# craabreu/openmm-nonbonded-slicing

Measured on AMD Instinct MI355X. Metric: ns/day (force evaluation only, dt = 2 fs), higher is better.
Workload: dtype f32

## Files before the change

### openmm-nonbonded-slicing_amd/csrc/engine.hip

```cpp
#include "../../include/snb.h"
#include "snb_internal.h"
#include "switches.h"
#include "host_lists.h"
#include "ewald_fit.h"
#include "pme_sizes.h"
#include "pair_addressing.h"

#include <algorithm>
#include <cstdio>
#include <cstdlib>
#include <chrono>
#include <cmath>
#include <cstring>
#include <map>
#include <numeric>
#include <set>
#include <thread>
#include <tuple>
#include <type_traits>

namespace snb {

static thread_local std::string g_createError;

// ... 138 lines not shown

static void bsplineModuli(int n, int order, std::vector<double>& out) {
    std::vector<double> data(order, 0.0), bsp(std::max(n, order + 1), 0.0);
    data[order - 1] = 0; data[1] = 0; data[0] = 1;
    for (int k = 3; k < order; k++) {
        double div = 1.0 / (k - 1.0);
        data[k - 1] = 0;
        for (int l = 1; l < (k - 1); l++) data[k - l - 1] = div * (l * data[k - l - 2] + (k - l) * data[k - l - 1]);
        data[0] = div * data[0];
    }
    double div = 1.0 / (order - 1);
    data[order - 1] = 0;
    for (int l = 1; l < (order - 1); l++) data[order - l - 1] = div * (l * data[order - l - 2] + (order - l) * data[order - l - 1]);
    data[0] = div * data[0];
    for (int i = 1; i <= order; i++) bsp[i] = data[i - 1];
    out.assign(n, 0.0);
    for (int i = 0; i < n; i++) {
        double sc = 0, ss = 0;
        for (int j = 0; j < n && j <= order; j++) { double arg = (2.0 * SNB_PI * i * j) / n; sc += bsp[j] * std::cos(arg); ss += bsp[j] * std::sin(arg); }
        out[i] = sc * sc + ss * ss;
    }
    for (int i = 0; i < n; i++)
        if (out[i] < 1.0e-7) out[i] = (out[(i - 1 + n) % n] + out[(i + 1) % n]) / 2;
}

template <typename Real> struct PmePlan {
    PmePlanDims d;
    double alpha = 0;
    bool dispersion = false;
    DevBuf<Real> gridReal;
    DevBuf<typename Vec<Real>::T2> gridCplx, gridCplxB, twx, twy, twz;
    DevBuf<Real> modx, mody, modz;
    DevBuf<Real> planeEterm; bool planeEtermReady = false, planeEtermFilled = false; double planeEtermKey[10] = {0};
    int ownSlabs = 0, ownMargin = 1; DevBuf<unsigned char> ownPartial; DevBuf<int> ownBusy; DevBuf<int2> strays;
    void init(const int g[3], int nGrids, hipStream_t s) {
        if (!planDims(g, sizeof(Real), switches(), d)) throw HipError{"PME mesh size is not FFT-legal"};
        if (d.nx > 1024 || d.ny > 1024 || d.nz > 1024) throw HipError{"PME mesh dimensions above 1024 are not supported"};
        gridReal.resize((size_t)nGrids * d.nx * d.ny * d.nz);
        gridCplx.resize((size_t)nGrids * d.nx * d.ny * d.nzc);
        if (planePath(d, nGrids, sizeof(Real), switches()).buffers) { gridCplxB.resize((size_t)nGrids * d.nx * (d.ny + 8) * d.nzc);
             planeEterm.resize((size_t)d.nx * d.ny * d.nzc); planeEtermReady = false; }
        auto tw = [&](int n, DevBuf<typename Vec<Real>::T2>& buf) {
            std::vector<typename Vec<Real>::T2> h(n);
            for (int k = 0; k < n; k++) { double a = -2.0 * SNB_PI * k / n; h[k].x = (Real)std::cos(a); h[k].y = (Real)std::sin(a); }
            buf.upload(h, s);
        };
        tw(d.nx, twx); tw(d.ny, twy); tw(d.nz, twz);
        auto md = [&](int n, DevBuf<Real>& buf) {
            std::vector<double> m; bsplineModuli(n, SNB_PME_ORDER, m);
            std::vector<Real> h(m.begin(), m.end());
            buf.upload(h, s);
        };
        md(d.nx, modx); md(d.ny, mody); md(d.nz, modz);
        HIPCHECK(hipStreamSynchronize(s));
    }
};

template <typename Real> class Engine : public EngineBase {
    using T4 = typename Vec<Real>::T4;
    using T2 = typename Vec<Real>::T2;
public:
    int N, nsub, S;
    hipStream_t stream = nullptr; bool ownStream = false;
    static constexpr int RING = 32;
    hipEvent_t evRebuild[3] = {nullptr, nullptr, nullptr};
    hipEvent_t evStepDone[2] = {nullptr, nullptr}; long long stepCounter = 0;
    hipStream_t stream2 = nullptr; hipEvent_t evFork = nullptr, evJoin = nullptr, evPairA = nullptr;
// ... 206 lines not shown
        HIPCHECK(hipHostMalloc((void**)&hNbPub, 64, hipHostMallocMapped));
        std::memset(hNbPub, 0, 64);
        HIPCHECK(hipHostGetDevicePointer((void**)&dNbPub, hNbPub, 0));
        for (int s = 0; s < nsub; s++) if (s % cfg.shard_count == cfg.shard_rank) ownedSubsets.push_back(s);
        nGrids = cfg.shard_count == 1 ? nsub : (int)ownedSubsets.size();
        if (isPme()) {
            for (int d = 0; d < 3; d++) cfg.grid[d] = legalGridSize(cfg.grid[d]);
            pme.alpha = cfg.alpha; pme.dispersion = false;
            if (nGrids > 0) pme.init(cfg.grid, nGrids, stream); else { pme.d.nx = cfg.grid[0]; pme.d.ny = cfg.grid[1]; pme.d.nz = cfg.grid[2]; }
            if (cfg.method == SNB_LJPME) {
                for (int d = 0; d < 3; d++) cfg.dgrid[d] = legalGridSize(cfg.dgrid[d]);
                dpme.alpha = cfg.alpha_d; dpme.dispersion = true;
                if (nGrids > 0) dpme.init(cfg.dgrid, nGrids, stream); else { dpme.d.nx = cfg.dgrid[0]; dpme.d.ny = cfg.dgrid[1]; dpme.d.nz = cfg.dgrid[2]; }
            }
            std::vector<int> gs = cfg.shard_count == 1 ? std::vector<int>() : ownedSubsets;
            if (cfg.shard_count == 1) { gs.resize(nsub); std::iota(gs.begin(), gs.end(), 0); }
            gridSubset.upload(gs, stream);
            hostGridSubset = gs;
        }
    }
    ~Engine() override {
        (void)hipStreamSynchronize(stream);
        if (sw.verbose && stats.n_rebuilds > 0) fprintf(stderr, "[snb] rebuilds: %lld, of them %lld built beside the steps; %lld side builds discarded\n", (long long)stats.n_rebuilds, sideBuilds, sideDiscarded);
        if (dStepTrace.p) {
            long long t[16] = {0}; (void)hipMemcpy(t, dStepTrace.p, sizeof(t), hipMemcpyDeviceToHost);
            auto us = [&](int k) { return t[k] ? (t[k] - t[0]) / 100.0 : -1.0; };
            fprintf(stderr, "[snb] step trace (us after the gather pass started; -1: not run): pair A %.1f .. %.1f | pair B %.1f .. %.1f | own %.1f | merge %.1f | plane %.1f | mix+z %.1f .. %.1f | interpolation %.1f .. %.1f\n",
                    us(2), us(3), us(4), us(5), us(6), us(7), us(8), us(9), us(10), us(11), us(12));
        }
        if (dPmeTrace.p) {
            long long g[8] = {0}; (void)hipMemcpy(g, dPmeTrace.p, 64, hipMemcpyDeviceToHost);
            if (g[7] > 0 && g[3] > 0) fprintf(stderr, "[snb] merge kernel prologue (busy flags, roots of unity, barrier): %.2f us per busy work-group\n", g[3] / 100.0 / g[7]);
            if (g[7] > 0) fprintf(stderr, "[snb] spreading (busy work-groups; scanning spreader: scan / entries / z FFT + store; merge kernel: sums / strays + z FFT / store): %.2f us, %.2f us, %.2f us per work-group (%lld work-groups)\n", g[4] / 100.0 / g[7], g[5] / 100.0 / g[7], g[6] / 100.0 / g[7], g[7]);
        }
        if (dPmeTrace.p) { long long h[4] = {0, 0, 0, 0}; (void)hipMemcpy(h, dPmeTrace.p, 32, hipMemcpyDeviceToHost); if (h[2] > 0) fprintf(stderr, "[snb] interpolation bricks: mean load %.2f us, mean compute %.2f us per work-group (%lld work-groups)\n", h[0] / 100.0 / h[2], h[1] / 100.0 / h[2], h[2]); }
        destroyGraphs();
        if (streamBuild) { (void)hipStreamSynchronize(streamBuild); (void)hipStreamDestroy(streamBuild); if (evSnap) (void)hipEventDestroy(evSnap); if (evBuilt) (void)hipEventDestroy(evBuilt); if (evFlagsReset) (void)hipEventDestroy(evFlagsReset); }
        if (streamCopy) { (void)hipStreamSynchronize(streamCopy); (void)hipStreamDestroy(streamCopy); }
        for (int k = 0; k < 2; k++) { if (evFrameStep[k]) (void)hipEventDestroy(evFrameStep[k]); if (evFrameUp[k]) (void)hipEventDestroy(evFrameUp[k]); if (framePinned[k]) (void)hipHostFree(framePinned[k]); }
        if (evBatchStart) (void)hipEventDestroy(evBatchStart);
        for (auto& g : sortGraphs) if (g.exec) (void)hipGraphExecDestroy(g.exec);
        sortGraphs.clear();
        for (auto& r : ring) { for (int k = 0; k < 5; k++) (void)hipEventDestroy(r.e[k]); for (int k = 0; k < 16; k++) { (void)hipEventDestroy(r.ks.start[k]); (void)hipEventDestroy(r.ks.stop[k]); } }
        for (int k = 0; k < 3; k++) if (evRebuild[k]) (void)hipEventDestroy(evRebuild[k]);
        for (int k = 0; k < 2; k++) if (evStepDone[k]) (void)hipEventDestroy(evStepDone[k]);
        if (hDispFlags) (void)hipHostFree(hDispFlags);
        if (hNbPub) (void)hipHostFree(hNbPub);
        if (stream2) { (void)hipEventDestroy(evFork); (void)hipEventDestroy(evJoin); (void)hipEventDestroy(evPairA); (void)hipStreamDestroy(stream2); }
        if (ownStream) (void)hipStreamDestroy(stream);
    }
    static constexpr int EW_DEG = sizeof(Real) == 4 ? 11 : SNB_EW_DEG_F64;
    static_assert(kEwaldFitLJPME == SNB_LJPME && kEwDegF32 == 11 && kEwDegF64 == SNB_EW_DEG_F64 && kDispDegF64 == SNB_DISP_DEG_F64, "ewald_fit.h and the kernels disagree");
    static_assert(kPolyForce == SNB_POLY_FORCE && kPolyEnergy == SNB_POLY_ENERGY && kPolyDispersion == SNB_POLY_DISPERSION, "ewald_fit.h and the kernels disagree");
    double ewPoly[EW_DEG + 1] = {0}; double ewPolyE[14] = {0}; double dispPoly[21] = {0}; double ewR2Max = 1;
    int polyMask = 0;
    void buildEwaldPoly() {
        const double rmax = cfg.cutoff + std::max(cfg.neighbor_padding, 0.0) + 0.02;
        const EwaldFit fit = fitEwaldPolys<Real>(cfg.alpha, cfg.alpha_d, cfg.cutoff, rmax, cfg.method);
        ewR2Max = fit.r2max;
        for (int i = 0; i <= EW_DEG; i++) ewPoly[i] = fit.ewPoly[i];
        for (int i = 0; i < 14; i++) ewPolyE[i] = fit.ewPolyE[i];
        for (int i = 0; i < 21; i++) dispPoly[i] = fit.dispPoly[i];
        const int have = sizeof(Real) == 4 ? (SNB_POLY_FORCE | SNB_POLY_ENERGY) : (SNB_POLY_FORCE | (cfg.method == SNB_LJPME ? SNB_POLY_DISPERSION : 0));
        polyMask = sw.ewaldErfc ? 0 : (sw.ewaldPolyAlways ? have : (fit.use & have));
        if (sw.verbose) fprintf(stderr, "[snb] Ewald polynomials: force max r|dBt| %.3g (limit %.3g), energy |dEt| %.3g (%.3g), dispersion max r|dGd| %.3g (%.3g): mask %d in use\n", fit.pairF, fit.limF, fit.sysE, fit.limE, fit.pairD, fit.limD, polyMask);
    }
// ... 511 lines not shown
            if (predicted && (h[7] > Npad || h[7] < N || (h[7] & 31))) {
                if (h[7] < N || (h[7] & 31)) throw HipError{"neighbour build: inconsistent padded atom count"};
                npadPredict = 0; padMispredictions++;
                if (sw.verbose) fprintf(stderr, "[snb] rebuild: padded count %d exceeded the predicted %d, repeating with the exact count (%lld so far)\n", h[7], Npad, (long long)padMispredictions);
                return gpuRebuild();
            }
            if (nbTrace && h[3] == 0) {
                std::vector<long long> tr((size_t)4 * numBlocks);
                HIPCHECK(hipMemcpy(tr.data(), dNbTrace.p, sizeof(long long) * tr.size(), hipMemcpyDeviceToHost));
                long long t0min = tr[0], t1max = tr[1]; std::vector<long long> dur(numBlocks);
                tr.resize((size_t)4 * numBlocks);
                for (int b = 0; b < numBlocks; b++) { t0min = std::min(t0min, tr[2 * b]); t1max = std::max(t1max, tr[2 * b + 1]); dur[b] = tr[2 * b + 1] - tr[2 * b]; }
                std::vector<long long> sorted = dur; std::sort(sorted.begin(), sorted.end());
                fprintf(stderr, "[snb] nb trace: span %.1f us; per-block duration median %.1f us, p90 %.1f, p99 %.1f, max %.1f us; last start at %.1f us\n", (t1max - t0min) / 100.0, sorted[numBlocks / 2] / 100.0,
                        sorted[numBlocks * 9 / 10] / 100.0, sorted[numBlocks * 99 / 100] / 100.0, sorted.back() / 100.0, (t1max - t0min) / 100.0);
                { std::vector<long long> a(numBlocks), b(numBlocks), c(numBlocks);
                  for (int k = 0; k < numBlocks; k++) { a[k] = tr[2 * numBlocks + 2 * k] - tr[2 * k]; b[k] = tr[2 * numBlocks + 2 * k + 1] - tr[2 * numBlocks + 2 * k]; c[k] = tr[2 * k + 1] - tr[2 * numBlocks + 2 * k + 1]; }
                  std::sort(a.begin(), a.end()); std::sort(b.begin(), b.end()); std::sort(c.begin(), c.end());
                  fprintf(stderr, "[snb] nb trace: median prologue %.1f us, gather %.1f us, final flush %.1f us\n", a[numBlocks / 2] / 100.0, b[numBlocks / 2] / 100.0, c[numBlocks / 2] / 100.0); }
                long long lastStart = 0; for (int b = 0; b < numBlocks; b++) lastStart = std::max(lastStart, tr[2 * b] - t0min);
                fprintf(stderr, "[snb] nb trace: last block start %.1f us after the first\n", lastStart / 100.0);
            }
            if (h[3] == 0) { acceptBuild(h, sortMs); gpuBuilt = true; needRebuild = false; paramsDirty = false; stepsSinceRebuild = 0; (void)t0; return true; }
            if (sw.verbose) fprintf(stderr, "[snb] gpu neighbour build attempt %d: tiles %d work %d masks %d overflow %d partial %d maxPartTiles %d maxPartWork %d (cap %zu, region %zu / %zu)\n", attempt, h[0], h[1], h[2], h[3], h[4], h[5], h[6], tileCap, tileCap / 64, (tileCap / 4 + 2 * numBlocks + 64) / 64);
            if ((size_t)h[5] > tileCap / 64 || (size_t)h[6] > (tileCap / 4 + 2 * numBlocks + 64) / 64) { tileCap = std::max((size_t)h[5] * 64 * 5 / 4, tileCap * 3 / 2) + 4096; continue; }
            return false;
        }
        return false;
    }

    void fillPme(PmeParams<Real>& p, PmePlan<Real>& plan, bool wantEnergy, const int* need, bool cellsReady = false, bool trace = false) {
        p.d = plan.d; p.nsub = nGrids; p.natoms = Npad; p.posq = posq.p; p.sigeps = sigeps.p; p.atomSubset = atomSubset.p; p.atomGrid = atomGrid.p;
        p.cells = pmeCells.p;
        if (sw.pmeTrace) { if (!dPmeTrace.p) { dPmeTrace.resize(8); HIPCHECK(hipMemset(dPmeTrace.p, 0, 64)); } p.trace = dPmeTrace.p; }
        p.stepTrace = (trace && plan.dispersion == (cfg.method == SNB_LJPME)) ? dStepTrace.p : nullptr;
        p.cellsReady = (!plan.dispersion && cellsReady) ? 1 : 0;
        p.fixDev = dFixScale.p ? dFixScale.p + (plan.dispersion ? 2 : 0) : nullptr;
        p.gridReal = plan.gridReal.p; p.gridCplx = plan.gridCplx.p; p.planeB = plan.gridCplxB.p; p.planeEterm = plan.planeEtermReady ? plan.planeEterm.p : nullptr; p.twx = plan.twx.p; p.twy = plan.twy.p; p.twz = plan.twz.p;
        p.modx = plan.modx.p; p.mody = plan.mody.p; p.modz = plan.modz.p;
        const double det = box[0] * box[4] * box[8];
        double r[9]; recipBoxRows(box, r);
        for (int i = 0; i < 9; i++) { p.recip[i] = (Real)r[i]; p.recipLo[i] = (Real)(r[i] - (double)p.recip[i]); }
        p.alpha = (Real)plan.alpha; p.volume = (Real)det; p.dispersion = plan.dispersion ? 1 : 0;
        p.lambdas = dLambdas.p; p.sliceNeed = need; p.gridSubset = gridSubset.p; p.emptyGrids = emptyGrids; p.nsubTotal = nsub; p.mix = cfg.shard_count == 1 ? 1 : 0;
        p.mix16 = sw.mix16 ? 1 : 0;
        p.sliceE = sliceE.p; p.fpx = fpx.p; p.fpy = fpy.p; p.fpz = fpz.p; p.wantEnergy = wantEnergy ? 1 : 0;
        p.sortNcx = p.sortNcy = 0; p.groupX = p.groupY = 1; p.colRange = nullptr;
        p.zSlabs = 1;
        if (plan.d.nz % 2 == 0 && plan.d.nz >= 32 && !(sizeof(Real) == 4)) p.zSlabs = 2;
        if (sw.zSlabs >= 1 && plan.d.nz % sw.zSlabs == 0) p.zSlabs = sw.zSlabs;
        const BrickGeometry b = bricksFor(plan);
        if (b.ok) {
            p.sortNcx = b.ncx; p.sortNcy = b.ncy; p.groupX = b.gx; p.groupY = b.gy; p.colRange = colRange.p;
            p.ownSlabs = plan.ownSlabs; p.ownMargin = plan.ownMargin; p.ownPartial = plan.ownPartial.p; p.ownBusy = plan.ownBusy.p;
            p.strays = plan.strays.p; p.strayCount = dStrayCount.p ? dStrayCount.p + (plan.dispersion ? 1 : 0) : nullptr;
            if (!p.ownPartial || !p.ownBusy || !p.strays || !p.strayCount) p.ownSlabs = 0;
        }
    }
    BrickGeometry bricksFor(const PmePlan<Real>& plan) const { return brickGeometry(plan.d, pme.d, colCells, sw.brickGroup); }
    void planPlaneTable(PmePlan<Real>& plan) {
        if (!plan.planeEterm.p || !plan.gridCplxB.p || nGrids <= 0) { plan.planeEtermReady = false; return; }
        double key[10]; for (int i = 0; i < 9; i++) key[i] = box[i]; key[9] = plan.alpha;
        if (plan.planeEtermReady && plan.planeEtermFilled && std::memcmp(key, plan.planeEtermKey, sizeof(key)) == 0) return;
        std::memcpy(plan.planeEtermKey, key, sizeof(key));
        plan.planeEtermReady = false;
        PmeParams<Real> pp; std::memset(&pp, 0, sizeof(pp));
        fillPme(pp, plan, false, dSliceNeedAll.p);
        plan.planeEtermFilled = launchPlaneEterm<Real>(pp, plan.planeEterm.p, stream);
        plan.planeEtermReady = true;
    }
    void describeMesh(const char* name, const PmePlan<Real>& plan) const {
        const BrickGeometry b = bricksFor(plan);
        const bool bricks = nGrids > 0 && b.ok;
        fprintf(stderr, "[snb] %s mesh %d x %d x %d: sort columns %d x %d of %d x %d cells, %s", name, plan.d.nx, plan.d.ny, plan.d.nz,
                colCells[0] > 0 ? pme.d.nx / colCells[0] : 0, colCells[0] > 0 ? pme.d.ny / colCells[1] : 0, colCells[0], colCells[1],
                !bricks ? "atomic spreader" : "");
        if (bricks) fprintf(stderr, "bricks of %d x %d columns, %s (slabs %d, margin %d)", b.gx, b.gy, plan.ownSlabs > 0 ? "own-atoms spreader planned" : "scanning brick spreader", plan.ownSlabs, plan.ownMargin);
        const PmePlanDims& d = plan.d;
        fprintf(stderr, "; fft splits x %d*%d y %d*%d z %d*%d, plane splits x %d*%d y %d*%d (%s)\n", d.rx1, d.rx2, d.ry1, d.ry2, d.rz1, d.rz2, d.px1, d.px2, d.py1, d.py2,
                (d.px1 <= 0 || d.py1 <= 0) ? "none" : planeIsStatic(d) ? "static" : "run-time");
    }
    void planOwnSpread(PmePlan<Real>& plan) {
        plan.ownSlabs = 0;
        const BrickGeometry b = bricksFor(plan);
        if (nGrids <= 0 || !b.ok) return;
        double r[9]; recipBoxRows(box, r);
        const int M = ownSpreadMargin(plan.d, r, cfg.neighbor_padding, sw);
        const OwnSpread o = ownSpread(plan.d, b, nGrids, sizeof(Real), M, sw);
        if (!o.slabs) return;
        plan.ownPartial.resize(o.partialBytes);
        plan.ownBusy.resize(o.regions); plan.strays.resize(std::max(Npad, 1));
        plan.ownSlabs = o.slabs; plan.ownMargin = M;
    }

    void checkBox(const double* x, bool recip, const std::string& prefix, bool kmax) {
        const double minAllowed = 1.999999 * cfg.cutoff;
        if (x && !(x[0] >= minAllowed && x[4] >= minAllowed && x[8] >= minAllowed)) { err = prefix + "The periodic box size has decreased to less than twice the nonbonded cutoff."; throw (int)SNB_ERR_BOX_TOO_SMALL; }
        if (cfg.method != SNB_Ewald || !recip) return;
        if (kmax && (cfg.kmax[0] < 1 || cfg.kmax[1] < 1 || cfg.kmax[2] < 1)) { err = "Ewald: kmax must be given explicitly (snb_config.kmax)"; throw (int)SNB_ERR_INVALID_ARGUMENT; }
        if (x && (x[3] != 0 || x[6] != 0 || x[7] != 0)) { err = prefix + "SlicedNonbondedForce: Ewald is not supported with non-rectangular boxes.  Use PME instead."; throw (int)SNB_ERR_UNSUPPORTED; }
    }
    bool beginExecute(bool forces, int includeRecip) {
        if (!haveParticles) throw HipError{"snb_execute: particles were not set"};
        if (!havePositions) throw HipError{"snb_execute: positions were not set"};
        if (isPeriodic()) {
            if (!haveBox) throw HipError{"snb_execute: box was not set"};
            checkBox(box, includeRecip != 0, "", true);
        }
        if (dLambdas.p == nullptr) setLambdas(lambdas.data());
        const bool autoMode = cfg.rebuild_interval < 0;
        if (autoMode && cfg.neighbor_padding > 0) {
            hipEvent_t& ev = evStepDone[stepCounter & 1];
            if (ev) HIPCHECK(hipEventSynchronize(ev));
        }
        if (flagsResetPending && hipEventQuery(evFlagsReset) == hipSuccess) flagsResetPending = false;
        const bool due = autoMode ? ((hDispFlags[0] != 0 && !flagsResetPending) || stepsSinceRebuild >= -cfg.rebuild_interval) : (cfg.rebuild_interval <= 1 || stepsSinceRebuild >= cfg.rebuild_interval);
        bool rebuilding = needRebuild || paramsDirty || due || cfg.neighbor_padding <= 0;
        if (!forces && rebuilding) keepLastForces();
        if (sidePending) {
            if (needRebuild || paramsDirty || staticDirty || valuesDirty || excValuesDirty || cfg.neighbor_padding <= 0) cancelSideBuild();
            else if (rebuilding && finishSideBuild()) rebuilding = false;
        }
        if ((valuesDirty || excValuesDirty) && !staticDirty && !rebuilding) refreshValues();
        if (rebuilding) { if (valuesDirty || excValuesDirty) { staticDirty = true; valuesDirty = excValuesDirty = false; } if (ctx.on) stageCtxPositions(ctxStage.p); rebuild(); }
// ... 978 lines not shown
```

### openmm-nonbonded-slicing_amd/csrc/pme.hip

```cpp
#include "snb_internal.h"
#include "switches.h"
#include "pme_sizes.h"
#include "pme_plan.h"
#include <cstdio>
#include <cstdlib>
#include <type_traits>
#include <algorithm>
#include <cstdlib>

namespace snb {

thread_local KernelStamps* g_stamps = nullptr;
template <typename Real> static inline int stampSlot(const PmeParams<Real>& p, int k) { return k + (p.dispersion ? 8 : 0); }

template <typename... KArgs, typename... Args>
static void launchLds(int slot, void (*kernel)(KArgs...), dim3 grid, dim3 block, size_t lds, hipStream_t s, const Args&... args) {
    hipFuncSetAttribute(reinterpret_cast<const void*>(kernel), hipFuncAttributeMaxDynamicSharedMemorySize, (int)lds);
    SNB_STAMPED_LAUNCH(slot, kernel, grid, block, lds, s, static_cast<KArgs>(args)...);
}
template <int A, int B, typename F> static void callPair(F& f) { f(std::integral_constant<int, A>{}, std::integral_constant<int, B>{}); }
template <typename F> static void forFftPair(int r1, int r2, F f) {
#define X(A, B) if (r1 == A && r2 == B) return callPair<A, B>(f);
    SNB_FFT_PAIRS(X)
#undef X
// ... 725 lines not shown
    Cx<Real>* A = reinterpret_cast<Cx<Real>*>(s_dyn);
    Cx<Real>* B = A + (size_t)nz * BS;
    Cx<Real>* tw = B + (size_t)nz * BS;
    __shared__ unsigned s_bmask[9];
    __shared__ int s_roff[9];
    __shared__ int s_any;
    const int loX = (4 + M + cx - 1) / cx, hiX = (M + cx - 1) / cx, loY = (4 + M + cy - 1) / cy, hiY = (M + cy - 1) / cy;
    if (tid == 0) s_any = 0;
    __syncthreads();
    if (tid < 9) {
        const int jy = tid / 3, jx = tid - jy * 3;
        const int dbx = jx - hiX, dby = jy - hiY;
        unsigned m = 0; int ro = 0;
        if (dbx <= loX && dby <= loY) {
            int bx2 = (Bx - dbx) % nbx; if (bx2 < 0) bx2 += nbx;
            int by2 = (By - dby) % nby; if (by2 < 0) by2 += nby;
            const int reg = ((slot * nbx + bx2) * nby + by2) * nSlabs;
            for (int sl = 0; sl < nSlabs; sl++) if (p.ownBusy[reg + sl]) m |= 1u << sl;
            ro = (int)((size_t)reg * npts) + (((jx - hiX) * cx + M) * RY + ((jy - hiY) * cy + M)) * RZ;
        }
        s_bmask[tid] = m; s_roff[tid] = ro;
        if (m) s_any = 1;
    }
    if (FUSEZ) for (int k = tid; k < nz; k += NT) tw[k] = reinterpret_cast<const Cx<Real>*>(p.twz)[k];
    const int nStray = *p.strayCount;
    const Real inv = FIXED ? p.fixDev[1] : Real(1);
    __syncthreads();
    long long trA = 0;
    if (trace) trA = wall_clock64();
    const Acc* partial = reinterpret_cast<const Acc*>(p.ownPartial);
    Real* greal = p.gridReal + (size_t)slot * nx * ny * nz;
    Cx<Real>* out = reinterpret_cast<Cx<Real>*>(p.gridCplx) + (size_t)slot * nx * ny * nzc;
    const FastDiv dzc(nzc), dcy2(cy);
    if (FUSEZ && !s_any && nStray == 0) {
        if (plane) {
            const FastDiv dnl(nl);
            for (int it = tid; it < nl * nzc; it += NT) {
                const int k = dnl.div(it), l = it - k * nl;
                out[((size_t)k * (nbx * nby) + bcol) * nl + l] = {Real(0), Real(0)};
            }
            return;
        }
        for (int it = tid; it < nl * nzc; it += NT) {
            const int l = dzc.div(it), k = it - l * nzc;
            const int lx = dcy2.div(l), ly = l - lx * cy;
            out[((size_t)(x0 + lx) * ny + (y0 + ly)) * nzc + k] = {Real(0), Real(0)};
        }
        return;
    }
    const int nch = nz / chunk;
    const int TPL = (NT / nl) > 0 ? (NT / nl) : 1, LPP = NT / TPL;
    const FastDiv dtpl(TPL);
    const int lineOfThread = dtpl.div(tid), sub = tid - lineOfThread * TPL;
    for (int l = lineOfThread; l < nl; l += LPP) {
        const int lx = dcy2.div(l), ly = l - lx * cy;
        const int lineOff = (lx * RY + ly) * RZ;
        unsigned okBits = 0;
#pragma unroll
        for (int jy = 0; jy < 3; jy++) {
            const int ry = ly + (jy - hiY) * cy + M;
#pragma unroll
            for (int jx = 0; jx < 3; jx++) {
                const int rx = lx + (jx - hiX) * cx + M;
                if (rx >= 0 && rx < RX && ry >= 0 && ry < RY) okBits |= 1u << (jy * 3 + jx);
            }
        }
// ... 551 lines not shown
            else for (int e0 = tid; e0 < (int)planeElems; e0 += 4 * NT) {
                float part = 0.f;
#pragma unroll
                for (int u = 0; u < 4; u++) {
                    const int e = e0 + u * NT;
                    if (e < (int)planeElems) { const Cx<Real> v = qc[e], a = P[tiledIndex(e)]; part += v.x * a.x + v.y * a.y; }
                }
                acc += (double)part;
            }
            acc *= (I == slot) ? 0.5 * w : w;
#pragma unroll
            for (int o = 32; o > 0; o >>= 1) acc += __shfl_xor(acc, o, 64);
            __syncthreads();
            if ((tid & 63) == 0) s_red[tid >> 6] = acc;
            __syncthreads();
            if (tid == 0) {
                double tot = 0; for (int k = 0; k < NT / 64; k++) tot += s_red[k];
                atomicAdd(&SNB_SLICE_E_PARTITION(p.sliceE, p.nsubTotal * (p.nsubTotal + 1))[2 * slice + term], tot);
            }
        }
    }
}

template <int R1, int R2, int NT> __global__ __launch_bounds__(NT) void k_fftZInvMix(const PmeParams<float> p, const int NBY) {
    SNB_PME_PRIO();
    SNB_TRACE_START(p.stepTrace, 9);
    using Real = float;
    typedef float f32x4 __attribute__((ext_vector_type(4)));
    const int nx = p.d.nx, ny = p.d.ny, nz = p.d.nz, nzc = p.d.nzc, nsub = p.nsub;
    const int NP = (nsub + 1) >> 1;
    const int tilesY = (ny + NBY - 1) / NBY;
    const int x = blockIdx.x / tilesY, y0 = (blockIdx.x - x * tilesY) * NBY;
    const int nby = (ny - y0) < NBY ? (ny - y0) : NBY;
    const int nb = nby * NP, BS = NBY * NP + 1;
    constexpr bool INPLACE = R1 > 0;
    Cx<Real>* A = reinterpret_cast<Cx<Real>*>(s_dyn);
    Cx<Real>* B = A + (INPLACE ? (size_t)0 : (size_t)nz * BS);
    Cx<Real>* tw = B + (size_t)nz * BS;
    const int tid = threadIdx.x, lane = tid & 63, wave = tid >> 6;
    for (int k = tid; k < nz; k += NT) tw[k] = reinterpret_cast<const Cx<Real>*>(p.twz)[k];
    const FastDiv dR1(INPLACE ? R1 : 1);
    auto zpos = [&](int k) { if constexpr (INPLACE) { const int k2 = dR1.div(k); return (k - k2 * R1) * R2 + k2; } else return k; };
    const int term = p.dispersion ? 1 : 0;
    float aReg[2][8];
#pragma unroll
    for (int g = 0; g < 2; g++)
#pragma unroll
        for (int J = 0; J < 8; J++) {
            const int I = 4 * g + (lane & 3);
            float v = 0.f;
            if (I < nsub && J < nsub) {
                if (p.mix) {
                    const int gi = p.gridSubset[I], gj = p.gridSubset[J];
                    v = p.lambdas[2 * (gi > gj ? gi * (gi + 1) / 2 + gj : gj * (gj + 1) / 2 + gi) + term];
                } else v = (I == J) ? 1.f : 0.f;
            }
            aReg[g][J] = v;
        }
    const size_t subStride = (size_t)nzc * NBY;
    const Cx<Real>* src = reinterpret_cast<const Cx<Real>*>(p.planeB) + (size_t)blockIdx.x * nsub * subStride;
    const int nPts = nzc * NBY;
    const FastDiv dNBY(NBY);
    const int nG = (nsub + 3) >> 2;
    for (int p0 = 64 * wave; p0 < nPts; p0 += NT) {
        const int pt = p0 + lane;
        const int kz = dNBY.div(pt < nPts ? pt : 0), yy = (pt < nPts ? pt : 0) - kz * NBY;
        const bool valid = pt < nPts && yy < nby;
        const Cx<Real>* s0 = src + (valid ? pt : 0);
        Cx<Real> v[8];
#pragma unroll
        for (int J = 0; J < 8; J++) { v[J] = {0.f, 0.f}; if (valid && J < nsub) v[J] = s0[J * subStride]; }
        f32x4 re[2], im[2];
#pragma unroll
        for (int g = 0; g < 2; g++) { re[g] = {0.f, 0.f, 0.f, 0.f}; im[g] = {0.f, 0.f, 0.f, 0.f}; }
#pragma unroll
        for (int g = 0; g < 2; g++) if (g < nG) {
#pragma unroll
            for (int J = 0; J < 8; J++) if (J < nsub) {
                re[g] = __builtin_amdgcn_mfma_f32_4x4x1f32(aReg[g][J], v[J].x, re[g], 0, 0, 0);
                im[g] = __builtin_amdgcn_mfma_f32_4x4x1f32(aReg[g][J], v[J].y, im[g], 0, 0, 0);
            }
        }
        if (valid) {
#pragma unroll
            for (int m = 0; m < 4; m++) if (m < NP) {
                const int g = m >> 1, r = (2 * m) & 3;
                const Cx<Real> a = {re[g][r], im[g][r]};
                Cx<Real> b = {0.f, 0.f};
                if (2 * m + 1 < nsub) b = {re[g][r + 1], im[g][r + 1]};
                const int c = yy * NP + m;
                A[zpos(kz) * BS + c] = {a.x - b.y, a.y + b.x};
                if (kz > 0 && nz - kz >= nzc) A[zpos(nz - kz) * BS + c] = {a.x + b.y, b.x - a.y};
            }
        }
    }
    Cx<Real>* R = A;
    if constexpr (INPLACE) {
        __syncthreads();
        planePass<Real, R2, +1, 0, false>(A, nb, 1, BS, R1, tw, tid, NT, PlaneNoScale());
        __syncthreads();
        planePass<Real, R1, +1, 2, true>(A, nb, 1, BS, R2, tw, tid, NT, PlaneNoScale());
    } else R = fftLines<Real, R1, R2>(A, B, nz, p.d.fz, p.d.nfz, +1, tw, nb, BS, tid, NT);
    __syncthreads();
    const FastDiv dz(nz), dnp(NP);
    for (int it = tid; it < nb * nz; it += NT) {
        const int c = dz.div(it), k = it - c * nz;
        const int yy = dnp.div(c), m = c - yy * NP;
        const Cx<Real> z = R[k * BS + c];
        p.gridReal[(((size_t)(2 * m) * nx + x) * ny + (y0 + yy)) * nz + k] = z.x;
        if (2 * m + 1 < nsub) p.gridReal[(((size_t)(2 * m + 1) * nx + x) * ny + (y0 + yy)) * nz + k] = z.y;
    }
    SNB_TRACE_END(p.stepTrace, 10);
}

static int fftyThreads() { return switches().fftThreads; }
template <typename Real, bool FWD> static void launchFftZ(const PmeParams<Real>& p, hipStream_t s) {
    const ZPass z = zPass(p.d.nz, sizeof(Real));
    const size_t nlines = (size_t)p.nsub * p.d.nx * p.d.ny;
    forFftPair(p.d.rz1, p.d.rz2, [&](auto A, auto B) {
        launchLds(stampSlot(p, FWD ? 2 : 6), &k_fftZ<Real, FWD, decltype(A)::value, decltype(B)::value>, dim3((unsigned)((nlines + z.NL - 1) / z.NL)), dim3(256), z.lds, s, p, z.NL);
    });
}
template <typename Real> static void launchFftStrided(int r1, int r2, const StridedPass& t, int batches, hipStream_t s, const PmeParams<Real>& p, int n, int lines, int sign, int axis) {
    forFftPair(r1, r2, [&](auto A, auto B) {
        launchLds(axis == 1 ? stampSlot(p, sign < 0 ? 3 : 5) : -1, &k_fftStrided<Real, decltype(A)::value, decltype(B)::value>, dim3((unsigned)(batches * t.tilesPerA)), dim3(fftyThreads()), t.lds, s,
                  p, n, (size_t)n * lines, lines, (size_t)lines, t.NB, t.tilesPerA, sign, axis);
    });
}
template <typename Real> static void launchFftY(const PmeParams<Real>& p, int sign, hipStream_t s) {
    launchFftStrided<Real>(p.d.ry1, p.d.ry2, yPass(p.d, sizeof(Real), switches()), p.nsub * p.d.nx, s, p, p.d.ny, p.d.nzc, sign, 1);
}

template <typename Real> static bool planePathOK(const PmeParams<Real>& p) { return p.planeB && p.planeEterm && planePath(p.d, p.nsub, sizeof(Real), switches()).ok; }
static void launchPlaneXY(const PmeParams<float>& p, hipStream_t s) {
    const PlanePath q = planePath(p.d, p.nsub, sizeof(float), switches());
    const int NBY = planeTileY(switches());
    const dim3 grid((unsigned)(p.nsub * p.d.nzc));
    const bool square = planeSquare(p.d, switches());
    if (p.energyOnly) {
        forPlanePair(square ? p.d.px1 : 0, square ? p.d.px2 : 0, [&](auto A, auto B) {
            launchLds(stampSlot(p, 4), &k_planeXY<decltype(A)::value, decltype(B)::value, 1024, true>, grid, dim3(1024), q.lds, s, p, NBY);
        });
        return;
// ... 433 lines not shown
```

### openmm-nonbonded-slicing_amd/csrc/pme_plan.h

```cpp
#pragma once
#include <algorithm>
#include <cmath>
#include <cstddef>

#include "switches.h"

#if defined(__HIPCC__)
#define SNB_PLAN_HD __host__ __device__
#else
#define SNB_PLAN_HD
#endif

namespace snb {

struct PmePlanDims {
    int nx, ny, nz, nzc;
    int nfx, nfy, nfz;
    int fx[16], fy[16], fz[16];
    int rx1, rx2, ry1, ry2, rz1, rz2;
    int px1, px2, py1, py2;
};

#ifndef SNB_FFT_120
#define SNB_FFT_120(X) X(10, 12)
// ... 102 lines not shown
    BrickGeometry b = bricksOf(d, ncx, ncy, gx, gy);
    b.ok = sizeof(double) * (size_t)b.cx * b.cy * d.nz <= 100 * 1024;
    return b;
}

inline int planeTileY(const Switches& sw) { return (sw.zmixNby == 2 || sw.zmixNby == 4 || sw.zmixNby == 8) ? sw.zmixNby : 8; }
struct PlanePath {
    size_t lds;
    bool buffers;
    bool ok;
    int threads;
};
inline PlanePath planePath(const PmePlanDims& d, int nsub, size_t realBytes, const Switches& sw) {
    PlanePath q;
    const bool square = planeSquare(d, sw);
    q.lds = 2 * realBytes * ((size_t)d.nx * (d.ny | 1) + d.nx + (square ? 0 : d.ny));
    q.buffers = realBytes == 4 && (size_t)d.nx * (d.ny | 1) * 8 <= 156 * 1024;
    q.ok = !sw.noPlaneFft && realBytes == 4 && !(d.ny & 1) && d.px1 > 0 && d.py1 > 0 && d.px1 * d.px2 == d.nx && d.py1 * d.py2 == d.ny
           && nsub <= 8 && q.lds <= 156 * 1024 && (square || !sw.noRectPlanes);
    q.threads = (square && sw.planeNt == 768) ? 768 : 1024;
    return q;
}

struct ZMix { int NBY; size_t lds; int threads; };
inline ZMix zMix(const PmePlanDims& d, int nsub, const Switches& sw) {
    ZMix z;
    const int NP = (nsub + 1) / 2;
    z.NBY = planeTileY(sw);
    const bool twoPass = isFftPair(d.rz1, d.rz2);
    z.lds = 8 * ((size_t)(twoPass ? 1 : 2) * d.nz * (z.NBY * NP + 1) + d.nz);
    const bool wide = sw.zmixNt ? sw.zmixNt == 512 : z.NBY * NP >= 24;
    z.threads = (wide && twoPass) ? 512 : 256;
    return z;
}

template <bool FIXED> SNB_PLAN_HD inline int ownLineStride(int RZ) {
    const int per = FIXED ? 4 : 2;
    int st = (RZ + per - 1) / per * per;
    while (((st * (FIXED ? 1 : 2)) & 7) != 4) st += per;
    return st;
}
inline int ownSpreadMargin(const PmePlanDims& d, const double r[9], double padding, const Switches& sw) {
    const double perNmX = d.nx * std::sqrt(r[0] * r[0] + r[3] * r[3] + r[6] * r[6]), perNmY = d.ny * std::sqrt(r[1] * r[1] + r[4] * r[4] + r[7] * r[7]);
    const int M = std::max(1, (int)std::ceil(0.5 * std::max(padding, 0.0) * std::max(perNmX, perNmY) + 0.01));
    return sw.spreadMargin >= 0 ? sw.spreadMargin : M;
}
struct OwnSpread {
    int slabs = 0;
    bool runs = false;
    bool fixed = false; size_t accBytes = 8;
    int RX = 0, RY = 0, RZ = 0;
    size_t regions = 0, partialBytes = 0;
    size_t ldsOwn = 0;
    int chunk = 1;
    int mergeThreads = 256;
    size_t ldsFft = 0; bool fuse = false;
    bool plane = false;
};
inline OwnSpread ownSpread(const PmePlanDims& d, const BrickGeometry& b, int nsub, size_t realBytes, int M, const Switches& sw) {
    OwnSpread o;
    o.fixed = realBytes == 4 && !sw.noFixedSpread;
    o.accBytes = o.fixed ? 4 : 8;
    const int cx = b.cx, cy = b.cy, nz = d.nz;
    const int RX = o.RX = cx + 4 + 2 * M, RY = o.RY = cy + 4 + 2 * M;
    if (RX > d.nx || RY > d.ny || b.gx * b.gy > 16 || nz > 256) return o;
    int best = 0;
// ... 106 lines not shown
```

### openmm-nonbonded-slicing_amd/csrc/snb_internal.h

```cpp
#pragma once
#include <hip/hip_runtime.h>
#include <hip/hip_ext.h>
#include <stdint.h>
#include <string>
#include <vector>

#include "pme_plan.h"

#define SNB_ONE_4PI_EPS0 138.93545764438198
#define SNB_PI 3.14159265358979323846
#define SNB_EPSILON0 (1.0 / (4.0 * SNB_PI * SNB_ONE_4PI_EPS0))
#define SNB_JIDX_MASK 0x01FFFFFF
#define SNB_JSHIFT_BITS 25
#define SNB_JCODE_CENTER 62
#define SNB_SLICE_E_PARTS 64
#define SNB_SLICE_E_PARTITION(base, stride) ((base) + (size_t)(blockIdx.x & (SNB_SLICE_E_PARTS - 1)) * (size_t)(stride))
#define SNB_PME_ORDER 5
#define SNB_TRACE_START(ptr, slot) do { if ((ptr) && blockIdx.x == 0 && threadIdx.x == 0) (ptr)[slot] = (long long)wall_clock64(); } while (0)
#define SNB_TRACE_END(ptr, slot) do { if ((ptr) && threadIdx.x == 0) (ptr)[slot] = (long long)wall_clock64(); } while (0)

#define SNB_EW_DEG_F64 16
#define SNB_DISP_DEG_F64 17
#define SNB_POLY_FORCE 1
#define SNB_POLY_ENERGY 2
// ... 144 lines not shown
    long long* stepTrace;
    long long* trace;
    int cellsReady;
    int* cells;
    Real* gridReal;
    typename Vec<Real>::T2* gridCplx;
    const Real* planeEterm;
    typename Vec<Real>::T2* planeB;
    const typename Vec<Real>::T2* twx; const typename Vec<Real>::T2* twy; const typename Vec<Real>::T2* twz;
    const Real* modx; const Real* mody; const Real* modz;
    Real recip[9];
    Real recipLo[9];
    Real alpha, volume;
    int dispersion;
    const Real* lambdas;
    const int* sliceNeed;
    const int* gridSubset;
    unsigned long long emptyGrids;
    int nsubTotal;
    int mix;
    int mix16;
    double* sliceE;
    Real* fpx; Real* fpy; Real* fpz;
    int wantEnergy;
    int sortNcx, sortNcy;
    int groupX, groupY;
    int zSlabs;
    const int2* colRange;
    int ownSlabs, ownMargin;
    void* ownPartial;
    int* ownBusy;
    int2* strays;
    int* strayCount;
    void* outForces; int outIsDouble, outAccumulate;
    const int* userToCtx; int ctxStride, ctxAtomic;
    EnergyOut finE;
    const double* finParts; double* finOut; int finN; SliceFinish fin;
    const Real* dfx; const Real* dfy; const Real* dfz; int dfs, dfixed;
    const int* sortedToUser;
    int energyOnly;
};

template <typename Real> struct EwaldParams {
    int natoms, nsub, nk;
    const typename Vec<Real>::T4* posq; const int* atomSubset;
    const int3* kvec;
    Real* cosSin;
    Real recipBox[3];
    double factorEwald, recipCoeff;
    const Real* lambdas; double* sliceE; int wantEnergy;
    Real* fpx; Real* fpy; Real* fpz;
};
template <typename Real> void launchEwald(const EwaldParams<Real>& p, hipStream_t s, bool forces = true);

template <typename Real> struct NbParams {
    int nAtoms, nPadded, nBlocks, nSubsets, subsetBits, colBits, ncx, ncy;
    double boxm[9];
    double origin[3];
    float listCutoff;
    int boxWalk;
    float jumpDist;
    const int* uSubset; const Real* uCharge; const typename Vec<Real>::T2* uSigEps;
    const int* uExclStart; const int* uExclList;
    const int* slotOfSubset;
    int* blockSubset;
    int* segKey; int* segStart; int* padExtra; int* padBefore;
// ... 155 lines not shown
```

### openmm-nonbonded-slicing_amd/csrc/switches.h

```cpp
#pragma once
#include <algorithm>
#include <cstdlib>

namespace snb {

struct Switches {
    static bool flag(const char* name) { return getenv(name) != nullptr; }
    static int intOr(const char* name, int unset) { const char* e = getenv(name); return e ? atoi(e) : unset; }
    static long long longOr(const char* name, long long unset) { const char* e = getenv(name); return e ? atoll(e) : unset; }
    static double realOr(const char* name, double unset) { const char* e = getenv(name); return e ? atof(e) : unset; }

    bool noOwnSpread = flag("SNB_NO_OWN_SPREAD");
    int ownSlabs = intOr("SNB_OWN_SLABS", 0);
    int spreadMargin = flag("SNB_SPREAD_MARGIN") ? std::max(0, intOr("SNB_SPREAD_MARGIN", 0)) : -1;
    bool noFusedZ = flag("SNB_NO_FUSED_Z");
    bool noFixedSpread = flag("SNB_NO_FIXED_SPREAD");
    int zSlabs = intOr("SNB_ZSLABS", 0);
    int brickGroup = intOr("SNB_BRICK_GROUP", 1);
    int mergeNt = intOr("SNB_MERGE_NT", 0);
    double fixHeadroom = realOr("SNB_FIX_HEADROOM", 0.0);
    bool fftTwoPass = intOr("SNB_FFT_TWOPASS", 1) != 0;
    int fftyNb = intOr("SNB_FFTY_NB", 0);
    int fftThreads = intOr("SNB_FFT_THREADS", 512) == 256 ? 256 : 512;
    int convLdsKB = intOr("SNB_CONV_LDS_KB", 72);
    bool planeDynamic = flag("SNB_PLANE_DYNAMIC");
    bool noRectPlanes = flag("SNB_NO_RECT_PLANES");
    bool convxStagedF64 = flag("SNB_CONVX_STAGED_F64");
    bool mix16 = flag("SNB_MIX_16X16");
    bool noPlaneFft = flag("SNB_NO_PLANE_FFT");
    int planeNt = intOr("SNB_PLANE_NT", 1024);
    int zmixNby = intOr("SNB_ZMIX_NBY", 0);
    int zmixNt = intOr("SNB_ZMIX_NT", 0);
    bool noInterpBricks = flag("SNB_NO_INTERP_BRICKS");
    int interpGroup = intOr("SNB_INTERP_GROUP", -1);
    int interpThreads = intOr("SNB_INTERP_THREADS", 0);
    int interpZSlabs = intOr("SNB_INTERP_ZSLABS", 0);
    bool ewaldErfc = flag("SNB_EWALD_ERFC");
    bool ewaldPolyAlways = flag("SNB_EWALD_POLY_ALWAYS");
    bool scalarEnergyKernel = flag("SNB_SCALAR_ENERGY_KERNEL");
    bool noFusedLists = flag("SNB_NO_FUSED_LISTS");
    int directWgs = intOr("SNB_DIRECT_WGS", 0);
    int itemTiles = std::max(1, std::min(32, intOr("SNB_ITEM_TILES", 8)));
    bool noStepGraph = flag("SNB_NO_STEP_GRAPH");
    bool noSortGraph = flag("SNB_NO_SORT_GRAPH");
    bool noFusedFinish = flag("SNB_NO_FUSED_FINISH");
    bool noFusedEnergyFinish = flag("SNB_NO_FUSED_ENERGY_FINISH");
    bool ctxAtomicAdd = flag("SNB_CTX_ATOMIC_ADD");
    bool concurrentPme = intOr("SNB_CONCURRENT_PME", 0) != 0;
    bool noKernelStamps = flag("SNB_NO_KERNEL_STAMPS");
    bool noPinnedRing = flag("SNB_NO_PINNED_RING");
    int overlap = intOr("SNB_OVERLAP", 1);
    long long overlapMinTiles = longOr("SNB_OVERLAP_MIN_TILES", 100000);
    int overlapCuLimit = intOr("SNB_OVERLAP_CU_LIMIT", 2);
    int overlapGridA = intOr("SNB_OVERLAP_GRID_A", 0);
    int overlapGridB = intOr("SNB_OVERLAP_GRID_B", 0);
    bool overlapByCount = flag("SNB_OVERLAP_BY_COUNT");
    bool overlapDebug = flag("SNB_OVERLAP_DEBUG");
    bool stepTrace = flag("SNB_STEP_TRACE");
    bool noGraphUpdate = flag("SNB_NO_GRAPH_UPDATE");
    bool eagerRebuildStep = flag("SNB_EAGER_REBUILD_STEP");
    bool pmePrioLow = flag("SNB_PME_PRIO_LOW");
    bool pmePrioHigh = flag("SNB_PME_PRIO_HIGH");
    bool hostTriclinic = flag("SNB_HOST_TRICLINIC");
    bool boxPrune = flag("SNB_BOX_PRUNE");
// ... 21 lines not shown
```

Measured before the change: 509.4.

## Skip inverse z FFT lines for sub-grids whose bricks held no charge

The spreading kernel records per brick and sub-grid whether any charge landed there. The inverse z-mix kernel reads these flags to build a mask of wanted sub-grids per tile. It then transforms only those lines, returning early when none are wanted, and packs y-pairs into complex lines rather than sub-grid pairs. This removes FFT and store work for empty sub-grid regions, at the cost of reading the busy flags and rewriting the column packing and indexing. Unwritten regions of gridReal are assumed to be consumed as zeros or ignored downstream.

```diff
diff --git a/openmm-nonbonded-slicing_amd/csrc/engine.hip b/openmm-nonbonded-slicing_amd/csrc/engine.hip
--- a/openmm-nonbonded-slicing_amd/csrc/engine.hip
+++ b/openmm-nonbonded-slicing_amd/csrc/engine.hip
@@ -194,7 +194,7 @@
     DevBuf<typename Vec<Real>::T2> gridCplx, gridCplxB, twx, twy, twz;
     DevBuf<Real> modx, mody, modz;
     DevBuf<Real> planeEterm; bool planeEtermReady = false, planeEtermFilled = false; double planeEtermKey[10] = {0};
-    int ownSlabs = 0, ownMargin = 1; DevBuf<unsigned char> ownPartial; DevBuf<int> ownBusy; DevBuf<int2> strays;
+    int ownSlabs = 0, ownMargin = 1; DevBuf<unsigned char> ownPartial; DevBuf<int> ownBusy, brickBusy; DevBuf<int2> strays;
     void init(const int g[3], int nGrids, hipStream_t s) {
         if (!planDims(g, sizeof(Real), switches(), d)) throw HipError{"PME mesh size is not FFT-legal"};
         if (d.nx > 1024 || d.ny > 1024 || d.nz > 1024) throw HipError{"PME mesh dimensions above 1024 are not supported"};
@@ -467,6 +467,11 @@
             long long g[8] = {0}; (void)hipMemcpy(g, dPmeTrace.p, 64, hipMemcpyDeviceToHost);
             if (g[7] > 0 && g[3] > 0) fprintf(stderr, "[snb] merge kernel prologue (busy flags, roots of unity, barrier): %.2f us per busy work-group\n", g[3] / 100.0 / g[7]);
             if (g[7] > 0) fprintf(stderr, "[snb] spreading (busy work-groups; scanning spreader: scan / entries / z FFT + store; merge kernel: sums / strays + z FFT / store): %.2f us, %.2f us, %.2f us per work-group (%lld work-groups)\n", g[4] / 100.0 / g[7], g[5] / 100.0 / g[7], g[6] / 100.0 / g[7], g[7]);
+        }
+        if (dPmeTrace.p) {
+            long long z[16] = {0}; (void)hipMemcpy(z, dPmeTrace.p + 8, sizeof(z), hipMemcpyDeviceToHost);
+            long long any = 0; for (int k = 0; k < 16; k++) any += z[k];
+            if (any > 0) { fprintf(stderr, "[snb] inverse z line pairs (transformed/skipped per slot):"); for (int k = 0; k < 8 && k < nGrids; k++) fprintf(stderr, " %lld/%lld", z[2 * k], z[2 * k + 1]); fprintf(stderr, "\n"); }
         }
         if (dPmeTrace.p) { long long h[4] = {0, 0, 0, 0}; (void)hipMemcpy(h, dPmeTrace.p, 32, hipMemcpyDeviceToHost); if (h[2] > 0) fprintf(stderr, "[snb] interpolation bricks: mean load %.2f us, mean compute %.2f us per work-group (%lld work-groups)\n", h[0] / 100.0 / h[2], h[1] / 100.0 / h[2], h[2]); }
         destroyGraphs();
@@ -1044,7 +1049,7 @@
     void fillPme(PmeParams<Real>& p, PmePlan<Real>& plan, bool wantEnergy, const int* need, bool cellsReady = false, bool trace = false) {
         p.d = plan.d; p.nsub = nGrids; p.natoms = Npad; p.posq = posq.p; p.sigeps = sigeps.p; p.atomSubset = atomSubset.p; p.atomGrid = atomGrid.p;
         p.cells = pmeCells.p;
-        if (sw.pmeTrace) { if (!dPmeTrace.p) { dPmeTrace.resize(8); HIPCHECK(hipMemset(dPmeTrace.p, 0, 64)); } p.trace = dPmeTrace.p; }
+        if (sw.pmeTrace) { if (!dPmeTrace.p) { dPmeTrace.resize(24); HIPCHECK(hipMemset(dPmeTrace.p, 0, 24 * sizeof(long long))); } p.trace = dPmeTrace.p; }
         p.stepTrace = (trace && plan.dispersion == (cfg.method == SNB_LJPME)) ? dStepTrace.p : nullptr;
         p.cellsReady = (!plan.dispersion && cellsReady) ? 1 : 0;
         p.fixDev = dFixScale.p ? dFixScale.p + (plan.dispersion ? 2 : 0) : nullptr;
@@ -1067,6 +1072,7 @@
             p.ownSlabs = plan.ownSlabs; p.ownMargin = plan.ownMargin; p.ownPartial = plan.ownPartial.p; p.ownBusy = plan.ownBusy.p;
             p.strays = plan.strays.p; p.strayCount = dStrayCount.p ? dStrayCount.p + (plan.dispersion ? 1 : 0) : nullptr;
             if (!p.ownPartial || !p.ownBusy || !p.strays || !p.strayCount) p.ownSlabs = 0;
+            p.brickBusy = (sw.zSkip && p.mix && p.ownSlabs > 0) ? plan.brickBusy.p : nullptr;
         }
     }
     BrickGeometry bricksFor(const PmePlan<Real>& plan) const { return brickGeometry(plan.d, pme.d, colCells, sw.brickGroup); }
@@ -1101,7 +1107,7 @@
         const OwnSpread o = ownSpread(plan.d, b, nGrids, sizeof(Real), M, sw);
         if (!o.slabs) return;
         plan.ownPartial.resize(o.partialBytes);
-        plan.ownBusy.resize(o.regions); plan.strays.resize(std::max(Npad, 1));
+        plan.ownBusy.resize(o.regions); plan.brickBusy.resize((size_t)nGrids * b.count()); plan.strays.resize(std::max(Npad, 1));
         plan.ownSlabs = o.slabs; plan.ownMargin = M;
     }
 
diff --git a/openmm-nonbonded-slicing_amd/csrc/pme.hip b/openmm-nonbonded-slicing_amd/csrc/pme.hip
--- a/openmm-nonbonded-slicing_amd/csrc/pme.hip
+++ b/openmm-nonbonded-slicing_amd/csrc/pme.hip
@@ -781,6 +781,7 @@
     Real* greal = p.gridReal + (size_t)slot * nx * ny * nz;
     Cx<Real>* out = reinterpret_cast<Cx<Real>*>(p.gridCplx) + (size_t)slot * nx * ny * nzc;
     const FastDiv dzc(nzc), dcy2(cy);
+    if (plane && p.brickBusy && tid == 0) p.brickBusy[blockIdx.x] = (s_any || nStray != 0) ? 1 : 0;
     if (FUSEZ && !s_any && nStray == 0) {
         if (plane) {
             const FastDiv dnl(nl);
@@ -1398,7 +1399,14 @@
     const int tilesY = (ny + NBY - 1) / NBY;
     const int x = blockIdx.x / tilesY, y0 = (blockIdx.x - x * tilesY) * NBY;
     const int nby = (ny - y0) < NBY ? (ny - y0) : NBY;
-    const int nb = nby * NP, BS = NBY * NP + 1;
+    const int half = nby >> 1;
+    const int BS = NBY * NP + 1;
+    const unsigned wanted = (unsigned)__builtin_amdgcn_readfirstlane((int)zTileWanted(zSkipBricks(nx, ny, p.sortNcx, p.sortNcy, p.groupX, p.groupY),
+                                                                                      p.mix ? p.brickBusy : nullptr, nsub, x, y0, nby));
+    const int nb = zPairCount(wanted, nby);
+    if (p.trace && threadIdx.x == 0)
+        for (int I = 0; I < nsub; I++) atomicAdd((unsigned long long*)&p.trace[8 + 2 * I + (((wanted >> I) & 1u) ? 0 : 1)], (unsigned long long)half);
+    if (wanted == 0) { SNB_TRACE_END(p.stepTrace, 10); return; }
     constexpr bool INPLACE = R1 > 0;
     Cx<Real>* A = reinterpret_cast<Cx<Real>*>(s_dyn);
     Cx<Real>* B = A + (INPLACE ? (size_t)0 : (size_t)nz * BS);
@@ -1447,17 +1455,16 @@
                 im[g] = __builtin_amdgcn_mfma_f32_4x4x1f32(aReg[g][J], v[J].y, im[g], 0, 0, 0);
             }
         }
-        if (valid) {
-#pragma unroll
-            for (int m = 0; m < 4; m++) if (m < NP) {
-                const int g = m >> 1, r = (2 * m) & 3;
-                const Cx<Real> a = {re[g][r], im[g][r]};
-                Cx<Real> b = {0.f, 0.f};
-                if (2 * m + 1 < nsub) b = {re[g][r + 1], im[g][r + 1]};
-                const int c = yy * NP + m;
-                A[zpos(kz) * BS + c] = {a.x - b.y, a.y + b.x};
-                if (kz > 0 && nz - kz >= nzc) A[zpos(nz - kz) * BS + c] = {a.x + b.y, b.x - a.y};
-            }
+        const bool odd = yy & 1;
+        const int zp = zpos(odd ? (kz > 0 ? nz - kz : 0) : kz) * BS + (yy >> 1);
+        const bool writes = valid && (!odd || (kz > 0 && nz - kz >= nzc));
+        int col = 0;
+#pragma unroll
+        for (int I = 0; I < 8; I++) if (I < nsub && ((wanted >> I) & 1u)) {
+            const Cx<Real> own = {re[I >> 2][I & 3], im[I >> 2][I & 3]};
+            const Cx<Real> oth = {__shfl_xor(own.x, 1, 64), __shfl_xor(own.y, 1, 64)};
+            if (writes) A[zp + col] = odd ? Cx<Real>{oth.x + own.y, own.x - oth.y} : Cx<Real>{own.x - oth.y, own.y + oth.x};
+            col += half;
         }
     }
     Cx<Real>* R = A;
@@ -1468,13 +1475,17 @@
         planePass<Real, R1, +1, 2, true>(A, nb, 1, BS, R2, tw, tid, NT, PlaneNoScale());
     } else R = fftLines<Real, R1, R2>(A, B, nz, p.d.fz, p.d.nfz, +1, tw, nb, BS, tid, NT);
     __syncthreads();
-    const FastDiv dz(nz), dnp(NP);
+    unsigned slotOf = 0;
+    { int w = 0; for (int I = 0; I < nsub; I++) if ((wanted >> I) & 1u) slotOf |= (unsigned)I << (4 * w++); }
+    const FastDiv dz(nz), dh(half);
     for (int it = tid; it < nb * nz; it += NT) {
         const int c = dz.div(it), k = it - c * nz;
-        const int yy = dnp.div(c), m = c - yy * NP;
+        const int w = dh.div(c), j = c - w * half;
+        const int I = (slotOf >> (4 * w)) & 15;
         const Cx<Real> z = R[k * BS + c];
-        p.gridReal[(((size_t)(2 * m) * nx + x) * ny + (y0 + yy)) * nz + k] = z.x;
-        if (2 * m + 1 < nsub) p.gridReal[(((size_t)(2 * m + 1) * nx + x) * ny + (y0 + yy)) * nz + k] = z.y;
+        Real* dst = p.gridReal + (((size_t)I * nx + x) * ny + (y0 + 2 * j)) * nz + k;
+        dst[0] = z.x;
+        dst[nz] = z.y;
     }
     SNB_TRACE_END(p.stepTrace, 10);
 }
diff --git a/openmm-nonbonded-slicing_amd/csrc/pme_plan.h b/openmm-nonbonded-slicing_amd/csrc/pme_plan.h
--- a/openmm-nonbonded-slicing_amd/csrc/pme_plan.h
+++ b/openmm-nonbonded-slicing_amd/csrc/pme_plan.h
@@ -158,6 +158,25 @@
     const bool wide = sw.zmixNt ? sw.zmixNt == 512 : z.NBY * NP >= 24;
     z.threads = (wide && twoPass) ? 512 : 256;
     return z;
+}
+
+struct ZSkipBricks { int cx, cy, nbx, nby; };
+SNB_PLAN_HD inline ZSkipBricks zSkipBricks(int nx, int ny, int ncx, int ncy, int gx, int gy) { return {gx * (nx / ncx), gy * (ny / ncy), ncx / gx, ncy / gy}; }
+inline ZSkipBricks zSkipBricks(const PmePlanDims& d, const BrickGeometry& b) { return zSkipBricks(d.nx, d.ny, b.ncx, b.ncy, b.gx, b.gy); }
+SNB_PLAN_HD inline unsigned zTileWanted(const ZSkipBricks& g, const int* brickBusy, int nsub, int x, int y0, int nby) {
+    const unsigned all = nsub >= 32 ? ~0u : ((1u << nsub) - 1u);
+    if (!brickBusy) return all;
+    const int bx = x / g.cx, byLo = y0 / g.cy, byHi = (y0 + nby - 1) / g.cy;
+    unsigned wanted = 0;
+    for (int I = 0; I < nsub; I++)
+        for (int by = byLo; by <= byHi; by++)
+            if (brickBusy[(I * g.nbx + bx) * g.nby + by]) wanted |= 1u << I;
+    return wanted;
+}
+SNB_PLAN_HD inline int zPairCount(unsigned wanted, int nby) { return __builtin_popcount(wanted) * (nby >> 1); }
+SNB_PLAN_HD inline int zPairColumn(unsigned wanted, int I, int j, int nby) {
+    if (!((wanted >> I) & 1u)) return -1;
+    return __builtin_popcount(wanted & ((1u << I) - 1u)) * (nby >> 1) + j;
 }
 
 template <bool FIXED> SNB_PLAN_HD inline int ownLineStride(int RZ) {
diff --git a/openmm-nonbonded-slicing_amd/csrc/snb_internal.h b/openmm-nonbonded-slicing_amd/csrc/snb_internal.h
--- a/openmm-nonbonded-slicing_amd/csrc/snb_internal.h
+++ b/openmm-nonbonded-slicing_amd/csrc/snb_internal.h
@@ -200,6 +200,7 @@
     int* ownBusy;
     int2* strays;
     int* strayCount;
+    int* brickBusy;
     void* outForces; int outIsDouble, outAccumulate;
     const int* userToCtx; int ctxStride, ctxAtomic;
     EnergyOut finE;
diff --git a/openmm-nonbonded-slicing_amd/csrc/switches.h b/openmm-nonbonded-slicing_amd/csrc/switches.h
--- a/openmm-nonbonded-slicing_amd/csrc/switches.h
+++ b/openmm-nonbonded-slicing_amd/csrc/switches.h
@@ -30,6 +30,7 @@
     bool noPlaneFft = flag("SNB_NO_PLANE_FFT");
     int planeNt = intOr("SNB_PLANE_NT", 1024);
     int zmixNby = intOr("SNB_ZMIX_NBY", 0);
+    bool zSkip = intOr("SNB_Z_SKIP", 1) != 0;
     int zmixNt = intOr("SNB_ZMIX_NT", 0);
     bool noInterpBricks = flag("SNB_NO_INTERP_BRICKS");
     int interpGroup = intOr("SNB_INTERP_GROUP", -1);
```

Result: no change. 513.0, median of 6 (+0.7%).
